# YoungSeng/QPGesture

Hardware: AMD Instinct MI355X
Metric: matched gesture frames/sec (GestureKNN) (higher is better)
Workload: dtype split-f16 products / f64 block sums + f64 re-evaluation; 1 GPU; 1 x 24 s clip (M=6 windows, Q=48 steps, 1440 frames each) per job vs speaker-10-class DB N_db=2048 windows (53248 candidates), shipped mode wavlm_feat(f32-bounded/f64-exact)+text(f32)+phase; n_db=2048, windows_per_clip=6, clips=1, clips_per_gpu=1, feature_dtype=f32, audio_precision=mixed, encode_batch=0, clips_in_flight=1, parallelism=single GPU, unsharded DB

## Files before the change

include/qpg.h:

```cpp
#ifndef QPG_H
#define QPG_H

#include <stddef.h>
#include <stdint.h>

#ifdef __cplusplus
extern "C" {
#endif

#define QPG_OK 0
#define QPG_EINVAL (-1)
#define QPG_EHIP (-2)
#define QPG_EUNSUP (-3)

typedef struct qpg_ctx qpg_ctx;

int qpg_version(void);
const char* qpg_build_id(void);
int qpg_ctx_create(int device, qpg_ctx** out);
int qpg_dev_kernarg(void);
int qpg_ctx_destroy(qpg_ctx* ctx);
#define QPG_OPT_GATE_DEDUP_FROM_CHAINS 0
#define QPG_OPT_TAKES_STAGES 1
#define QPG_OPT_NOPHASE_STAGES 2
// ... 113 lines not shown
                           int16_t* out_rank, int q_block, int64_t block_stride);
int qpg_percode_select_f32(qpg_ctx*, void* stream, const float* D, int64_t ldD, int Q, const int16_t* cand_code,
                           int64_t C, int K, float absent, int32_t idx_base, float* out_dist, int32_t* out_idx,
                           int16_t* out_rank, int q_block, int64_t block_stride);

int qpg_percode_select_guarded_f64(qpg_ctx*, void* stream, const double* D, int64_t ldD, int Q, const int16_t* cand_code,
                                   int64_t C, int K, double absent, int32_t idx_base, double* out_dist, int32_t* out_idx,
                                   int16_t* out_rank, int q_block, int64_t block_stride, const float* base, int T, int F,
                                   const int32_t* cand_t, int G, int n_taps, int tap_stride, const float* q32, double eps,
                                   int32_t* stats, int base_is_f16);

int64_t qpg_percode_select_exact_ws_bytes(int Q, int64_t C, int K);
int qpg_percode_select_exact_f64(qpg_ctx*, void* stream, const double* D, int64_t ldD, int Q, const int16_t* cand_code,
                                 int64_t C, int K, double absent, int32_t idx_base, double* out_dist, int32_t* out_idx,
                                 int16_t* out_rank, int q_block, int64_t block_stride, const float* base, int T, int F,
                                 const int32_t* cand_t, int G, int n_taps, int tap_stride, const float* q32, double eps,
                                 int32_t* stats, int base_is_f16, void* ws, int64_t ws_bytes);

int qpg_percode_select_mixed_f64(qpg_ctx*, void* stream, const void* D, int d_is_f32, int64_t ldD, int Q, const int16_t* cand_code,
                                 int64_t C, int K, double absent, int32_t idx_base, double* out_dist, int32_t* out_idx,
                                 int16_t* out_rank, int q_block, int64_t block_stride, const float* base, int T, int F,
                                 const int32_t* cand_t, int G, int n_taps, int tap_stride, const float* q32,
                                 const double* qn2, const double* cn2, double eps1, double eps2, int32_t* stats,
                                 void* ws, int64_t ws_bytes, int base_is_f16);
int64_t qpg_percode_select_mixed_ws_bytes(int Q, int K);
int64_t qpg_percode_select_mixed_ws_stride(int K);
int qpg_percode_select_mixed_f64_cut(qpg_ctx*, void* stream, const void* D, int d_is_f32, int64_t ldD, int Q,
                                     const int16_t* cand_code, int64_t C, int K, double absent, int32_t idx_base,
                                     double* out_dist, int32_t* out_idx, int16_t* out_rank, int q_block, int64_t block_stride,
                                     const float* base, int T, int F, const int32_t* cand_t, int G, int n_taps,
                                     int tap_stride, const float* q32, const double* qn2, const double* cn2, double eps1,
                                     double eps2, int32_t* stats, void* ws, int64_t ws_bytes, int base_is_f16,
                                     const int16_t* pos_rank_t, const int16_t* freq_rank, int top_n, int probe);

int64_t qpg_merge_mixed_ws_bytes(int Q, int K, int fl_cap);
int qpg_merge_mixed_phase1_f64(qpg_ctx*, void* stream, const void* recv, int W, int64_t src_stride, int64_t dist_off,
                               int64_t idx_off, int Q, int K, double absent, double eps1, int R, void* req,
                               int64_t req_stride, void* ws, int64_t ws_bytes, int32_t* stats, int fl_cap,
                               int64_t flag_off);
int qpg_shard_refine_f64(qpg_ctx*, void* stream, const void* req_recv, int W, int64_t req_stride, int R, int q_stride,
                         int64_t cand_base, const float* base, int base_is_f16, int T, int F, const int32_t* cand_t, int G,
                         int n_taps, int tap_stride, const float* q32, const double* qn2, const double* cn2, void* resp,
                         int64_t resp_stride, int reference_arithmetic, int32_t* stats, int Rq);
int qpg_flags_stamp(qpg_ctx*, void* stream, void* buf, int nblk, int64_t stride, int64_t off, const int32_t* stats);
int qpg_flags_gather(qpg_ctx*, void* stream, const void* buf, int nblk, int64_t stride, int64_t off, int32_t* stats);
int qpg_merge_mixed_phase2_f64(qpg_ctx*, void* stream, const void* recv, int W, int64_t src_stride, int64_t idx_off, int Q,
                               int K, double absent, const void* ws, int64_t ws_bytes, const void* resp_recv,
                               int64_t resp_stride, double* out_dist, int32_t* out_idx, int16_t* out_rank, int32_t* stats,
                               int fl_cap, double eps2);

int qpg_merge_select_f64(qpg_ctx*, void* stream, const void* recv, int W, int64_t src_stride, int64_t dist_off,
                         int64_t idx_off, int Q, int K, double absent, double* out_dist, int32_t* out_idx,
                         int16_t* out_rank, double eps2, int32_t* stats);
int qpg_merge_select_f32(qpg_ctx*, void* stream, const void* recv, int W, int64_t src_stride, int64_t dist_off,
                         int64_t idx_off, int Q, int K, float absent, float* out_dist, int32_t* out_idx,
                         int16_t* out_rank);

int qpg_rank_rows_f64(qpg_ctx*, void* stream, const double* d, int Q, int K, int16_t* out);
int qpg_rank_rows_f32(qpg_ctx*, void* stream, const float* d, int Q, int K, int16_t* out);


int qpg_l2_table_f32(qpg_ctx*, void* stream, const float* sig, int K, int Dm, float* out);

#define QPG_MODE_AUD_TXT 0
#define QPG_MODE_AUD 1
#define QPG_MODE_TXT 2
// ... 338 lines not shown
```

qpgesture_amd/code_knn.py:

```python
import ctypes
from collections import namedtuple
from typing import NamedTuple, Optional

import numpy as np
import torch

from . import _lib
from .parallel import allreduce_max_, allreduce_min_index, exchange_bytes, shard_rows
from .sorted_rows import SortedRows

from .constant import (ABSENT_DIST, NUM_AUDIO_FEAT_FRAMES, STEP_SZ, WAVVQ_GROUP_SIZE, codebook_size, num_frames,
                       num_frames_code)

MODE_AUD_TXT, MODE_AUD, MODE_TXT = _lib.QPG_MODE_AUD_TXT, _lib.QPG_MODE_AUD, _lib.QPG_MODE_TXT
AUDIO_MX_ERR = _lib.QPG_AUDIO_MX_ERR
AUDIO_MX_BAND = 2.1 * AUDIO_MX_ERR
AUDIO_HL_ERR = _lib.QPG_AUDIO_HL_ERR
AUDIO_HL_BAND = 2.1 * AUDIO_HL_ERR

FLAG_LIST_OVERFLOW, FLAG_SMALL_NORMS, FLAG_REQUEST_OVERFLOW, FLAG_CROSS_SHARD_TIE = 1, 2, 4, 8
FLAG_TEXT_OVERFLOW = 16


_PIN_SENTINEL = -1234567
# ... 227 lines not shown
        from . import db_cache
        return db_cache.save(self, path, key, sources=sources)

    @classmethod
    def load(cls, path, device="cuda:0", key=None):
        from . import db_cache
        dev = torch.device(device)
        if dev.type != "cuda":
            raise RuntimeError("GestureDB needs a HIP device (got %s); there is no CPU path" % dev)
        _lib.load()
        db = db_cache.load(path, dev, key)
        if db is None:
            return None
        if db.hl_image is not None or db.txt_sorted is not None:
            from .selfcheck import mfma_bound_ok
            db.hl_bound_ok, db.hl_bound_report = mfma_bound_ok(dev)
            if not db.hl_bound_ok:
                db.hl_image = db.txt_sorted = None
        return db

    @staticmethod
    def _cand_code(code_local, cidx, dev):
        cc = np.ascontiguousarray(code_local[:, np.asarray(cidx, np.int64)].reshape(-1))
        cc = np.where((cc >= 0) & (cc < 32767), cc, -1).astype(np.int16)
        return torch.from_numpy(cc if cc.size else np.zeros((1,), np.int16)).to(dev)

    @property
    def idx_base(self):
        return self.lo


Knobs = namedtuple("Knobs", "audio_precision audio_kernel text_kernel tie_eps mixed_single_launch sharded_mixed "
                   "sharded_mixed_min_gflop force_sharded overlap_sweeps text_after_sweep audio_first fused_pack rank_cut "
                   "split_fuse split_fuse_max_steps host_ranks use_wavvq",
                   defaults=("mixed", "hl", "mfma", 1e-12, False, True, 20.0, False, True, True, None, True, True, True,
                             256, False, False))
DBFacts = namedtuple("DBFacts", "n_local N world K Ga F Dt feature_dtype hl_bound_ok has_hl_image has_txt_sorted hl_planes",
                     defaults=("f32", True, True, True, 2))


class AudioPlan(NamedTuple):
    path: str
    kernel: str
    band: float
    cut_top_n: int
    fused_rank: bool


class StepPlan(NamedTuple):
    audio: Optional[AudioPlan]
    text: Optional[str]
    sharded: bool
    exchange: Optional[str]
    clip_pack: bool
    split_fuse: bool
    overlap: bool
    order: Optional[str]


def plan_audio(kn, db, Q, want_rank=False, reduce=True, out_given=False, cut_top_n=0):
    C = db.n_local * db.Ga
    fused_rank = want_rank and db.world == 1
    local_final = fused_rank and reduce and not out_given
    shard_part = (db.world > 1 or kn.force_sharded) and not reduce and out_given
    gflop = 2e-9 * Q * (-(-db.N // db.world) * db.Ga) * NUM_AUDIO_FEAT_FRAMES * db.F
    guard = kn.tie_eps > 0 and C > 0
    half = db.feature_dtype == "f16"
    if (kn.audio_precision == "mixed" and guard and db.K <= 512 and db.hl_bound_ok and
            (local_final or (shard_part and kn.sharded_mixed and gflop >= kn.sharded_mixed_min_gflop))):
        hl = kn.audio_kernel == "hl" and db.has_hl_image
        kernel = ("hl" if db.hl_planes == 2 else "hl1") if hl else ("mx_h" if half else "mx")
        cut = cut_top_n if (cut_top_n in (1, 2) and local_final and not kn.mixed_single_launch) else 0
        return AudioPlan("mixed", kernel, AUDIO_HL_BAND if hl else AUDIO_MX_BAND, cut, fused_rank)
    path = "exact" if (kn.audio_precision == "exact" and guard) else ("guarded" if guard else "plain")
    return AudioPlan(path, "f64_h" if half else "f64", 0.0, 0, fused_rank)


def plan_text(kn, db, Q, reduce=True, out_given=False):
    mfma = (kn.text_kernel == "mfma" and db.has_txt_sorted and Q > 0 and kn.audio_precision != "exact" and
            ((not out_given and reduce and db.world == 1) or (out_given and not reduce)))
    return "mfma" if mfma else "valu"


def plan_step(kn, db, M, steps, mode=MODE_AUD_TXT, for_walk=False, owner_blocks=False):
    Q = M * steps
    sharded = db.world > 1 or kn.force_sharded
    audio = text = None
    if mode != MODE_TXT and not kn.use_wavvq:
        cut = 0
        if for_walk and kn.rank_cut and not sharded and not kn.host_ranks:
            cut = 1 if mode == MODE_AUD_TXT else 2
        audio = plan_audio(kn, db, Q, want_rank=not sharded, reduce=not sharded, out_given=sharded, cut_top_n=cut)
    if mode != MODE_AUD:
        text = plan_text(kn, db, Q, reduce=not sharded, out_given=sharded)
    split = (for_walk and mode == MODE_AUD_TXT and not sharded and not kn.host_ranks and kn.split_fuse and
             db.K % 16 == 0 and db.K <= 4096 and Q <= kn.split_fuse_max_steps)
    overlap = mode == MODE_AUD_TXT and kn.overlap_sweeps
    mfma_text = kn.text_kernel == "mfma" and db.has_txt_sorted and kn.audio_precision != "exact"
    clip_pack = (overlap and not kn.use_wavvq and mfma_text and audio.kernel in ("hl", "hl1") and db.Dt % 128 == 0 and
                 kn.fused_pack)
    audio_first = mfma_text if kn.audio_first is None else bool(kn.audio_first)
    after = overlap and kn.text_after_sweep and not audio_first and not kn.use_wavvq
    order = None
    if overlap:
        order = "audio_first" if audio_first else ("text_after_sweep" if after else "text_first")
    exchange = ("all_to_all" if owner_blocks else "all_gather") if sharded else None
    return StepPlan(audio, text, sharded, exchange, clip_pack, split, overlap, order)

# ... 62 lines not shown
        if use_wavvq and not db.has_wavvq:
            raise ValueError("GestureDB was built without a wavvq track")
        self.db = db
        self.use_wavvq = use_wavvq
        if use_wavvq:
            self.step_sz, self.n_db_frm = db.vq_step, db.Tv
        else:
            self.step_sz, self.n_db_frm = db.step_sz, db.T
        self.n_db_seq = db.N
        self.use_phase, self.use_txt = use_phase, use_txt
        if not use_phase and not 0 <= int(desired_k) < _lib.QPG_NOPHASE_KMAX:
            raise ValueError("desired_k must be in [0, %d) (got %r)" % (_lib.QPG_NOPHASE_KMAX, desired_k))
        self.desired_k = int(desired_k)
        self.last_picks = None
        self.rng = rng if rng is not None else np.random
        self.overlap_sweeps = True
        self.text_after_sweep = True
        self.audio_first = None
        self.serial_walk = False
        self.tie_eps = 1e-12
        self._guard_stats = torch.zeros((4,), dtype=torch.int32, device=db.device)
        self.audio_precision = "mixed"
        self.audio_kernel = "hl"
        self.text_kernel = "mfma"
        self._txt_scratch = {}
        self.fallbacks = 0
        import os as _os
        self.fused_pack = _os.environ.get("QPG_FUSED_PACK", "1") != "0"
        self.rank_cut = _os.environ.get("QPG_RANK_CUT", "1") != "0"
        self.rank_cut_probe = 64
        self.mixed_single_launch = False
        self.split_fuse = True
        self.split_fuse_max_steps = 256
        self.sharded_mixed = True
        self.force_sharded = False
        self.sharded_mixed_min_gflop = 20.0
        self.mixed_requests = None
        self.host_ranks = False

        self._qpos, self._qcache, self._layouts, self._mm_cache, self._pinned_ints, self._plans = None, {}, {}, {}, {}, {}
        self._side_stream = self._side_gate = self._side_done = self._sweep_event = None
        self._mix_ws = self._exact_ws = self._hl_qimage = self._takes_ws = self._nophase_ws = None
        self._pinned_nophase = None
        self.kernel_events, self.kernel_events_every, self.kernel_event_pool, self._ev_calls = None, 1, None, 0
        self.text_fallbacks, self.tables, self._last_mix_Q = 0, None, 0
        self._last_audio_mixed = self._last_audio_exact = self._last_audio_hl = False
        self._last_text_mfma = self._last_rank_cut = False
        self._last_D_aud = self._last_q32 = self._last_qn2 = self._last_ints = self._last_gate_tables = None

    def _knobs(self):
        return Knobs(self.audio_precision, self.audio_kernel, self.text_kernel, self.tie_eps, self.mixed_single_launch,
                     self.sharded_mixed, self.sharded_mixed_min_gflop, self.force_sharded, self.overlap_sweeps,
                     self.text_after_sweep, self.audio_first, self.fused_pack, self.rank_cut, self.split_fuse,
                     self.split_fuse_max_steps, self.host_ranks, self.use_wavvq)

    def _facts(self):
        db = self.db
        return DBFacts(db.n_local, db.N, db.world, db.K, db.Ga, db.F, db.Dt, db.feature_dtype, db.hl_bound_ok,
                       db.hl_image is not None, db.txt_sorted is not None, db.hl_planes)

    def _audio_grid(self):
        db = self.db
        if self.use_wavvq:
            return db.vq_cidx, db.vq_pslot, db.Gv
        return db.aud_cidx, db.aud_pslot, db.Ga

    def query_positions(self):
        key = (self.n_db_frm, self.step_sz)
        if self._qpos is not None and self._qpos[0] == key:
            return self._qpos[1]
        pos, i = [], 0
        while i < self.n_db_frm:
            pos.append(i)
            i += STEP_SZ * self.step_sz
        self._qpos = (key, pos)
        return pos

    def init_code_phase(self):
        db = self.db
        i = self.rng.randint(0, self.n_db_seq)
        j = self.rng.randint(0, self.n_db_frm - int(num_frames / num_frames_code))
        code = int(db.code_host[i, j // num_frames_code])
        if not self.use_phase:
            return code
        P = db.phase_host[i, j:j + 8]
        if P.shape[0] != 8:
            raise ValueError("init_code_phase drew frame %d: phase slice has %d rows, not 8 "
# ... 65 lines not shown
        else:
            assert prepacked is None, "the one-launch clip pack feeds the split-f16 sweep only"
            _lib.call("qpg_audio_pack_queries", dev, qbase, M, T, F, _i32(q_win, dev), _i32(q_t, dev), Q,
                      NUM_AUDIO_FEAT_FRAMES, ts, q32, qn2)
        if timer is not None:
            timer[0].record(torch.cuda.current_stream(dev))
        if use_hl:
            sweep_launch()
        else:
            strides = (1, D.stride(0), self._guard_stats) if mixed else (D.stride(0),)
            _lib.call(sweep_fn, dev, db.base, db.n_local, db.T, db.F, db.aud_t, db.Ga, NUM_AUDIO_FEAT_FRAMES,
                      db.tap_stride, db.cn2, q32, qn2, Q, D, *strides)
        if timer is not None:
            timer[1].record(torch.cuda.current_stream(dev))
            self.kernel_events.append(timer)
        if after_sweep is not None:
            after_sweep()
        if sweep_event is not None:
            sweep_event.record(torch.cuda.current_stream(dev))
        if plan.path == "plain":
            dist, idx, rank = self._select_plain(D, db.aud_cand_code, C, db.Ga, out, plan.fused_rank)
        else:
            dist, idx, rank, qb, bs = self._tables_out(Q, torch.float64, out, plan.fused_rank)
            tables = (Q, db.aud_cand_code, C, db.K, float(ABSENT_DIST), db.idx_base * db.Ga, dist, idx, rank, qb, bs)
            track = (db.base, db.T, db.F, db.aud_t, db.Ga, NUM_AUDIO_FEAT_FRAMES, db.tap_stride, q32)
        if mixed:
            ws = self._mix_ws = _grown(self._mix_ws, int(_lib.load().qpg_percode_select_mixed_ws_bytes(Q, db.K)), dev,
                                       zero=True)
            single = self.mixed_single_launch
            sel_args = (D, 1, D.stride(0), *tables, *track, qn2, db.cn2, plan.band, float(self.tie_eps),
                        self._guard_stats, None if single else ws, 0 if single else ws.numel(), int(half))
            try:
                if plan.cut_top_n:
                    _lib.call("qpg_percode_select_mixed_f64_cut", dev, *sel_args, db.pos_rank_t, db.freq_rank,
                              int(plan.cut_top_n), int(self.rank_cut_probe))
                else:
                    _lib.call("qpg_percode_select_mixed_f64", dev, *sel_args)
            except Exception:
                self._mix_ws = None
                raise
        elif plan.path == "exact":
            ws = self._exact_ws = _grown(self._exact_ws, int(_lib.load().qpg_percode_select_exact_ws_bytes(Q, C, db.K)),
                                         dev)
            _lib.call("qpg_percode_select_exact_f64", dev, D, D.stride(0), *tables, *track, float(self.tie_eps),
                      self._guard_stats, int(half), ws, ws.numel())
        elif plan.path == "guarded":
            _lib.call("qpg_percode_select_guarded_f64", dev, D, D.stride(0), *tables, *track, float(self.tie_eps),
                      self._guard_stats, int(half))
        self._last_audio_mixed, self._last_audio_exact, self._last_audio_hl = mixed, plan.path == "exact", use_hl
        self._last_rank_cut, self._last_D_aud, self._last_q32, self._last_qn2 = plan.cut_top_n > 0, D, q32, qn2
        if mixed:
            self._last_mix_Q = Q
        return AudioResult(dist, idx, rank, D, q32, qn2, plan)

    def sweep_text(self, queries, want_rank=False, reduce=True, normalised=False, out=None, cols_packed=False, kind=None):
        db, dev = self.db, self.db.device
        Q = queries.shape[0]
        if normalised:
            qn = queries
        else:
            qn = torch.empty_like(queries)
            _lib.call("qpg_l2_normalize_rows_f32", dev, queries, Q, db.Dt, qn)
        if kind is None:
            kind = plan_text(self._knobs(), self._facts(), Q, reduce, out is not None)
        self._last_text_mfma = kind == "mfma"
        if kind == "mfma":
            dist, idx, rank, qb, bs = self._tables_out(Q, torch.float32, out, want_rank and out is None)
            db.txt_sorted.select(qn, float(ABSENT_DIST), self._guard_stats, dist=dist, idx=idx, rank=rank,
# ... 579 lines not shown
```

qpgesture_amd/csrc/qpg_select.hip:

```cpp
#include "qpg_common.h"

__device__ __forceinline__ unsigned long long order_key(double d) {
  unsigned long long b = (unsigned long long)__double_as_longlong(d);
  return (b >> 63) ? ~b : (b | 0x8000000000000000ull);
}
__device__ __forceinline__ double key_value(unsigned long long k, double) {
  unsigned long long b = (k >> 63) ? (k & 0x7fffffffffffffffull) : ~k;
  return __longlong_as_double((long long)b);
}
__device__ __forceinline__ unsigned int order_key(float d) {
  unsigned int b = __float_as_uint(d);
  return (b >> 31) ? ~b : (b | 0x80000000u);
}
__device__ __forceinline__ float key_value(unsigned int k, float) {
  unsigned int b = (k >> 31) ? (k & 0x7fffffffu) : ~k;
  return __uint_as_float(b);
}

template <typename T, typename KeyT, bool PACKED>
__global__ __launch_bounds__(1024) void percode_select_kernel(const T* __restrict__ D, int64_t ldD,
                                                              const int16_t* __restrict__ cand_code, int64_t C, int K,
                                                              T absent, int32_t idx_base, T* __restrict__ out_dist,
                                                              int32_t* __restrict__ out_idx,
                                                              int16_t* __restrict__ out_rank, int q_block,
// ... 392 lines not shown
      [&]() {
        if (tid == 0) A.stats[1] = 1;
      },
      rank_pass);
}

extern "C" int qpg_percode_select_guarded_f64(qpg_ctx* ctx, void* stream, const double* D, int64_t ldD, int Q,
                                              const int16_t* cand_code, int64_t C, int K, double absent,
                                              int32_t idx_base, double* out_dist, int32_t* out_idx, int16_t* out_rank,
                                              int q_block, int64_t block_stride, const float* base, int T, int F,
                                              const int32_t* cand_t, int G, int n_taps, int tap_stride,
                                              const float* q32, double eps, int32_t* stats, int base_is_f16) {
  const char* name = "qpg_percode_select_guarded_f64";
  QPG_REQUIRE(ctx && D && (cand_code || C == 0) && out_dist && out_idx && base && cand_t && q32 && stats,
              "%s: null pointer", name);
  QPG_REQUIRE(Q >= 0 && C >= 0 && K > 0 && K <= 2048 && ldD >= C && C + (int64_t)idx_base < 0x7fffffffll && eps >= 0.0,
              "%s: bad size (K <= 2048)", name);
  QPG_REQUIRE(select_block_layout_ok(q_block, block_stride, Q, out_rank), QPG_BLOCK_LAYOUT_MSG, name);
  GuardArgs A;
  if (int rc = guard_args(name, &A, base, base_is_f16, q32, cand_t, T, F, G, n_taps, tap_stride, C, eps, stats)) return rc;
  if (Q == 0) return QPG_OK;
  size_t sh = 24 * (size_t)K + GUARD_LIST * 16 + 16;
  const int sort_ranks = sh + 12 * (size_t)rank_sort_pow2(K) <= 64 * 1024;
  if (sort_ranks) sh += 12 * (size_t)rank_sort_pow2(K);
  hipLaunchKernelGGL(percode_select_guarded_f64_kernel, dim3(Q), dim3(1024), sh, qpg_stream(stream), D, ldD, cand_code,
                     C, K, absent, idx_base, out_dist, out_idx, out_rank, q_block, block_stride, A, sort_ranks);
  QPG_LAUNCH_CHECK("percode_select_guarded_f64_kernel");
  return QPG_OK;
}

#define MIX_LIST 2048
#define MIX_LIST2 256
#define MIX_POT 6144

template <int NPER>
__device__ __forceinline__ double pair_dot_fast_f64(const GuardArgs& A, const float* qlds, int64_t c_local, int lane) {
  const int j = (int)(c_local / A.G), g = (int)(c_local - (int64_t)j * A.G);
  const int t0 = A.cand_t[g];
  const int64_t crow = (int64_t)j * A.T * A.F + lane * 4;
  f32x4 cv[6][NPER];
#pragma unroll
  for (int tap = 0; tap < 6; ++tap) {
    const int t = t0 + tap * A.tap_stride;
    const bool ok = t < A.T;
    const int64_t cp = crow + (int64_t)(ok ? t : t0) * A.F;
#pragma unroll
    for (int u = 0; u < NPER; ++u) {
      cv[tap][u] = guard_val4(A, cp + 256 * u);
      if (!ok) cv[tap][u] = (f32x4){0.f, 0.f, 0.f, 0.f};
    }
  }
  double s0 = 0.0, s1 = 0.0;
#pragma unroll
  for (int tap = 0; tap < 6; ++tap)
#pragma unroll
    for (int u = 0; u < NPER; ++u) {
      const f32x4 qv = *reinterpret_cast<const f32x4*>(qlds + tap * A.F + 256 * u + lane * 4);
      s0 += (double)qv.x * (double)cv[tap][u].x;
      s1 += (double)qv.y * (double)cv[tap][u].y;
      s0 += (double)qv.z * (double)cv[tap][u].z;
      s1 += (double)qv.w * (double)cv[tap][u].w;
    }
  double s = s0 + s1;
  for (int o = 32; o > 0; o >>= 1) s += __shfl_xor(s, o, 64);
  return s;
}
// ... 157 lines not shown
        if (key[u][e] < o) o = atomicMin(&best32[code], key[u][e]);
        const unsigned int lo = o < key[u][e] ? o : key[u][e];
        if ((double)d[u][e] <= (double)key_value(lo, 0.f) + eps1) {
          const int pp = atomicAdd(&n_pot, 1);
          if (pp < MIX_SPOT) {
            pc[pp] = (int)(b + (int64_t)u * blockDim.x * 4 + e);
            pd[pp] = d[u][e];
            pk[pp] = (int16_t)code;
          }
        }
      }
  }
  for (int64_t c = cv + tid; c < c1; c += blockDim.x) visit(c, row[c], cand_code[c]);
  __syncthreads();
  MixStream m = mix_stream_of(ws, q, K);
  for (int k = tid; k < K; k += blockDim.x) m.inv[(size_t)sl * K + k] = ~best32[k];
  const int np = n_pot;
  if (np > MIX_SPOT) {
    if (tid == 0) m.cnt[sl] = -1;
    return;
  }
  const int seg = sl * MIX_SPOT;
  for (int e = tid; e < np; e += blockDim.x) {
    if (!((double)pd[e] <= (double)key_value(best32[pk[e]], 0.f) + eps1)) continue;
    const int pos = seg + atomicAdd(&n_keep, 1);
    m.pot_c[pos] = pc[e];
    m.pot_d[pos] = pd[e];
    m.pot_k[pos] = pk[e];
  }
  __syncthreads();
  if (tid == 0) m.cnt[sl] = n_keep;
}

template <typename DT>
__global__ __launch_bounds__(1024) void percode_select_mixed_f64_kernel(
    const DT* __restrict__ D, int64_t ldD, const int16_t* __restrict__ cand_code, int64_t C, int K, double absent,
    int32_t idx_base, double* __restrict__ out_dist, int32_t* __restrict__ out_idx, int16_t* __restrict__ out_rank,
    int q_block, int64_t block_stride, GuardArgs A, double eps1, const double* __restrict__ cn2,
    const double* __restrict__ qn2, int use_qlds, int phase, unsigned char* __restrict__ ws, int pre, RankCut RC) {
  extern __shared__ __attribute__((aligned(16))) unsigned char smem[];
  unsigned long long* best = reinterpret_cast<unsigned long long*>(smem);
  double* v = reinterpret_cast<double*>(smem + 8 * (size_t)K);
  unsigned int* besti = reinterpret_cast<unsigned int*>(smem + 16 * (size_t)K);
  unsigned int* near_ = besti + K;
  int* s_code = reinterpret_cast<int*>(near_ + K);
  unsigned char* refd = reinterpret_cast<unsigned char*>(s_code + K);
  unsigned char* tail = smem + 32 * (size_t)K;
  double* l_d = reinterpret_cast<double*>(tail);
  int* l_c = reinterpret_cast<int*>(tail + 8 * MIX_LIST);
  int* l_k = l_c + MIX_LIST;
  int* l2 = l_k + MIX_LIST;
  int* ctl = l2 + MIX_LIST2;
  int* p_c = ctl + 8;
  int16_t* p_k = reinterpret_cast<int16_t*>(p_c + MIX_LIST);
  int* rk = reinterpret_cast<int*>(p_k + MIX_LIST);
  int* pot_c = rk + K;
  int16_t* pot_k = reinterpret_cast<int16_t*>(pot_c + MIX_POT);
  float* qlds = reinterpret_cast<float*>(pot_k + MIX_POT);
  const int q = blockIdx.x, tid = threadIdx.x, lane = tid & 63, wv = tid >> 6, nwv = blockDim.x >> 6;
  const DT* row = D + (int64_t)q * ldD;
  select_out_rows(q, K, q_block, block_stride, out_dist, out_idx);
  unsigned char* wq = ws ? mix_query_base(ws, q, K) : nullptr;
  for (int k = tid; k < K; k += blockDim.x) {
    best[k] = ~0ull;
    besti[k] = 0xffffffffu;
    near_[k] = 0;
    refd[k] = 0;
// ... 138 lines not shown
    for (int e = tid; e < npot; e += blockDim.x) pass2(pot_c[e], (double)row[pot_c[e]], pot_k[e]);
  } else {
#pragma unroll 4
    for (int64_t c = (int64_t)tid * VE; c < Cv; c += (int64_t)blockDim.x * VE) {
      const vecD d = *reinterpret_cast<const vecD*>(row + c);
      const vecC cd = *reinterpret_cast<const vecC*>(cand_code + c);
#pragma unroll
      for (int e = 0; e < VE; ++e) pass2(c + e, (double)d[e], cd[e]);
    }
    for (int64_t c = Cv + tid; c < C; c += blockDim.x) pass2(c, (double)row[c], cand_code[c]);
  }
  __syncthreads();
  if (streamed && tid < MIX_SPLIT) ms.cnt[tid] = 0;
  for (int k = tid; k < K; k += blockDim.x) v[k] = besti[k] != 0xffffffffu ? key_value(best[k], 0.0) : absent;
  __syncthreads();
  const bool cut = RC.pos_t != nullptr && streamed && out_rank != nullptr && phase == 1;
  unsigned char* need2 = nullptr;
  if (cut) {
    unsigned char* cs = reinterpret_cast<unsigned char*>(pot_c);
    const int Kp = rank_sort_pow2(K);
    unsigned long long* skey2 = reinterpret_cast<unsigned long long*>(cs);
    int* scode2 = reinterpret_cast<int*>(skey2 + Kp);
    int16_t* lo_ = reinterpret_cast<int16_t*>(scode2 + Kp);
    int16_t* hi_ = lo_ + K;
    unsigned char* need = reinterpret_cast<unsigned char*>(hi_ + K);
    need2 = need + K;
    double* red = reinterpret_cast<double*>(cs + 12 * (size_t)Kp + 8 * (size_t)((K + 7) / 8 * 8));
    const double f05 = tid < K ? (double)RC.freq[tid] * 0.05 : 0.0;
    block_sorted_ranks(v, K, skey2, scode2, [&](int k, int r) {
      s_code[r] = k;
      rk[k] = r;
    });
    __syncthreads();
    for (int r = tid; r < K; r += blockDim.x) reinterpret_cast<int16_t*>(wq + mix_park_order_off(K))[r] = (int16_t)s_code[r];
    order_parked = true;
    for (int r = tid; r < K; r += blockDim.x) {
      const int k = s_code[r];
      int b = 0, a = 0;
      if (besti[k] != 0xffffffffu) {
        while (r - 1 - b >= 0 && v[k] - v[s_code[r - 1 - b]] <= eps1) ++b;
        while (r + 1 + a < K && besti[s_code[r + 1 + a]] != 0xffffffffu && v[s_code[r + 1 + a]] - v[k] <= eps1) ++a;
      }
      lo_[k] = (int16_t)(r - b);
      hi_[k] = (int16_t)(r + a);
    }
    __syncthreads();
    int np = RC.probe < K ? RC.probe : K;
    np = np < 64 ? np : 64;
    double* pf_ = red + 17;
    double* ph_ = pf_ + 64;
    int* pk_ = reinterpret_cast<int*>(ph_ + 64);
    double* pm_ = reinterpret_cast<double*>(pk_ + 64);
    if (tid < K) pm_[tid] = f05;
    __syncthreads();
    for (int r = tid; r < 64; r += blockDim.x) {
      const int k = r < np ? s_code[r] : -1;
      const bool ok = k >= 0 && besti[k] != 0xffffffffu;
      pk_[r] = ok ? k : -1;
      pf_[r] = ok ? pm_[k] : 0.0;
      ph_[r] = ok ? (double)hi_[k] : 0.0;
    }
    __syncthreads();
    double u = -1.0, m1 = __builtin_inf(), m2 = __builtin_inf();
    const int pp = tid < K ? tid : tid - K, half = tid < K ? 0 : 1;
    if (tid < 2 * K) {
      const int r0 = 32 * half;
      int kk[32];
// ... 108 lines not shown
      const long long b = (long long)floor(v[k] * inv_w);
      const unsigned int s0 = slot(b);
      bool company = false;
#pragma unroll
      for (int o = -1; o <= 1; ++o) {
        const unsigned int si = slot(b + o);
        if (o != 0 && si == s0) continue;
        unsigned int c = cell[si];
        if (si == s0) c -= 0x10000u + (unsigned int)k;
        const unsigned int pop = c >> 16;
        if (pop == 1) {
          const int other = (int)(c & 0xffffu);
          company |= fabs(v[other] - v[k]) < eps1;
        } else if (pop > 1) {
          company = true;
        }
      }
      if (!company || (need2 && !need2[k])) continue;
      if (atomicMax(&near_[k], 2u) >= 2u) continue;
      const int pos = atomicAdd(&ctl[0], 1);
      if (pos < MIX_LIST) {
        l_c[pos] = (int)(besti[k] - (unsigned int)idx_base);
        l_k[pos] = k;
      }
    }
    __syncthreads();
  }
  n = ctl[0];
  if (n > MIX_LIST) {
    n = MIX_LIST;
    if (tid == 0) atomicOr(&A.stats[1], 1);
  }
  }
  if (phase == 1) {
    unsigned long long* w_best = reinterpret_cast<unsigned long long*>(wq);
    double* w_v = reinterpret_cast<double*>(wq + 8 * (size_t)K);
    unsigned int* w_bi = reinterpret_cast<unsigned int*>(wq + 16 * (size_t)K);
    unsigned int* w_nr = w_bi + K;
    int* w_n = reinterpret_cast<int*>(wq + 24 * (size_t)K);
    int* w_lc = w_n + 4;
    int* w_lk = w_lc + MIX_LIST;
    for (int k = tid; k < K; k += blockDim.x) {
      w_best[k] = best[k];
      w_v[k] = v[k];
      w_bi[k] = besti[k];
      w_nr[k] = near_[k];
    }
    for (int e = tid; e < n; e += blockDim.x) {
      w_lc[e] = l_c[e];
      w_lk[e] = l_k[e];
    }
    if (tid == 0) {
      w_n[0] = n;
      w_n[1] = order_parked ? 1 : 0;
    }
    return;
  }
  if (phase == 2) {
    const unsigned long long* w_best = reinterpret_cast<const unsigned long long*>(wq);
    const double* w_v = reinterpret_cast<const double*>(wq + 8 * (size_t)K);
    const unsigned int* w_bi = reinterpret_cast<const unsigned int*>(wq + 16 * (size_t)K);
    const unsigned int* w_nr = w_bi + K;
    const int* w_n = reinterpret_cast<const int*>(wq + 24 * (size_t)K);
    const int* w_lc = w_n + 4;
    const int* w_lk = w_lc + MIX_LIST;
    const double* w_ld = reinterpret_cast<const double*>(w_lk + MIX_LIST);
    n = w_n[0];
    for (int k = tid; k < K; k += blockDim.x) {
      best[k] = w_best[k];
      v[k] = w_v[k];
      besti[k] = w_bi[k];
      near_[k] = w_nr[k];
    }
    for (int e = tid; e < n; e += blockDim.x) {
      l_c[e] = w_lc[e];
      l_k[e] = w_lk[e];
      l_d[e] = w_ld[e];
    }
    if (RC.pos_t) {
      unsigned char* isref = reinterpret_cast<unsigned char*>(pot_c);
      for (int k = tid; k < K; k += blockDim.x) isref[k] = 0;
      __syncthreads();
      for (int e = tid; e < n; e += blockDim.x) isref[w_lk[e]] = 1;
    }
    __syncthreads();
  }
  if (n > 0) {
    const double qq = qn2[q];
    const bool fast = use_qlds != 0;
    if (phase == 0 && fast) {
      const int D4 = (A.n_taps * A.F) >> 2;
      const f32x4* src = reinterpret_cast<const f32x4*>(A.q32 + (int64_t)q * A.n_taps * A.F);
      for (int i = tid; i < D4; i += blockDim.x) reinterpret_cast<f32x4*>(qlds)[i] = src[i];
      __syncthreads();
    }
    for (int e = wv; e < n && phase == 0; e += nwv) {
      const double d = pair_distance_wave(A, q, qlds, l_c[e], lane, fast, qq, cn2);
      if (lane == 0) l_d[e] = d;
    }
    for (int k = tid; k < K; k += blockDim.x)
      if (near_[k] >= 2) {
        rk[k] = (int)besti[k];
        best[k] = ~0ull;
        besti[k] = 0xffffffffu;
        s_code[k] = 0;
      }
    __syncthreads();
    for (int e = tid; e < n; e += blockDim.x) atomicMin(&best[l_k[e]], (unsigned long long)order_key(l_d[e]));
    __syncthreads();
    if (A.eps > 0.0) {
      for (int e = tid; e < n; e += blockDim.x)
        if (l_d[e] <= key_value(best[l_k[e]], 0.0) + A.eps) atomicAdd(&s_code[l_k[e]], 1);
      __syncthreads();
      for (int e = tid; e < n; e += blockDim.x)
        if (s_code[l_k[e]] >= 2 && l_d[e] <= key_value(best[l_k[e]], 0.0) + A.eps) {
          const int pos = atomicAdd(&ctl[2], 1);
          if (pos < MIX_LIST2) l2[pos] = e;
        }
      __syncthreads();
      int n2 = ctl[2];
      if (n2 > MIX_LIST2) {
        n2 = MIX_LIST2;
        if (tid == 0) atomicOr(&A.stats[1], 1);
      }
      if (n2 > 0) {
        for (int i0 = 0; i0 < n2; i0 += blockDim.x / 4) {
          const int i = i0 + (tid >> 2);
          const int e = l2[i < n2 ? i : 0];
          const double dr = refine_pair_f64(A, q, l_c[e], tid & 3);
// ... 3 lines not shown
          }
        }
        __syncthreads();
        for (int k = tid; k < K; k += blockDim.x)
          if (refd[k]) best[k] = ~0ull;
        __syncthreads();
        for (int i = tid; i < n2; i += blockDim.x)
          atomicMin(&best[l_k[l2[i]]], (unsigned long long)order_key(l_d[l2[i]]));
        __syncthreads();
        if (tid == 0) atomicAdd(&A.stats[0], n2);
      }
    }
    for (int e = tid; e < n; e += blockDim.x)
      if ((unsigned long long)order_key(l_d[e]) == best[l_k[e]])
        atomicMin(&besti[l_k[e]], (unsigned int)(l_c[e] + idx_base));
    __syncthreads();
    for (int k = tid; k < K; k += blockDim.x)
      if (near_[k] >= 2) {
        if (best[k] != ~0ull) v[k] = key_value(best[k], 0.0);
        else besti[k] = (unsigned int)rk[k];
      }
    if (tid == 0) atomicAdd(&A.stats[2], n);
    __syncthreads();
  }
  for (int k = tid; k < K; k += blockDim.x) {
    const bool have = besti[k] != 0xffffffffu;
    out_dist[(int64_t)q * K + k] = v[k];
    out_idx[(int64_t)q * K + k] = have ? (int32_t)besti[k] : -1;
  }
  if (!out_rank) return;
  if (tid == 0) ctl[2] = 0;
  __syncthreads();
  bool repaired = false;
  if (phase == 2 && RC.pos_t && reinterpret_cast<const int*>(wq + 24 * (size_t)K)[1] == 1) {
    const int16_t* w_order = reinterpret_cast<const int16_t*>(wq + mix_park_order_off(K));
    for (int r = tid; r < K; r += blockDim.x) s_code[r] = w_order[r];
    __syncthreads();
    for (int round = 0; round < 24 && !repaired; ++round) {
      if (tid == 0) ctl[5] = 0;
      __syncthreads();
#pragma unroll
      for (int parity = 0; parity < 2; ++parity) {
        for (int r = 2 * tid + parity; r + 1 < K; r += 2 * blockDim.x) {
          const int ka = s_code[r], kb = s_code[r + 1];
          if (rank_gt(rank_sort_key(v[ka]), ka, rank_sort_key(v[kb]), kb)) {
            s_code[r] = kb;
            s_code[r + 1] = ka;
            ctl[5] = 1;
          }
        }
        __syncthreads();
      }
      repaired = ctl[5] == 0;
      __syncthreads();
    }
    if (repaired)
      for (int r = tid; r < K; r += blockDim.x) out_rank[(int64_t)q * K + s_code[r]] = (int16_t)r;
  }
  if (!repaired) rank_pass(true);
  if (A.eps <= 0.0) return;
  __syncthreads();
  for (int r = tid; r + 1 < K; r += blockDim.x) {
    const int ka = s_code[r], kb = s_code[r + 1];
    if (besti[ka] == 0xffffffffu || besti[kb] == 0xffffffffu) continue;
    if (phase == 2 && RC.pos_t &&
        !(reinterpret_cast<const unsigned char*>(pot_c)[ka] && reinterpret_cast<const unsigned char*>(pot_c)[kb]))
      continue;
    if (v[kb] - v[ka] < A.eps) {
#pragma unroll
      for (int h = 0; h < 2; ++h) {
        const int k = h ? kb : ka;
        if (atomicExch(&near_[k], 0xffffffffu) == 0xffffffffu || refd[k]) continue;
        const int pos = atomicAdd(&ctl[2], 1);
        if (pos < MIX_LIST2) {
          l2[pos] = k;
        }
      }
    }
  }
  __syncthreads();
  int n3 = ctl[2];
  if (n3 == 0) return;
  if (n3 > MIX_LIST2) {
    n3 = MIX_LIST2;
    if (tid == 0) atomicOr(&A.stats[1], 1);
  }
  for (int i0 = 0; i0 < n3; i0 += blockDim.x / 4) {
    const int i = i0 + (tid >> 2);
    const int k = l2[i < n3 ? i : 0];
    const double dr = refine_pair_f64(A, q, (int64_t)(besti[k] - (unsigned int)idx_base), tid & 3);
    if (i < n3 && (tid & 3) == 0) {
      v[k] = dr;
      out_dist[(int64_t)q * K + k] = dr;
    }
  }
  if (tid == 0) atomicAdd(&A.stats[0], n3);
  __syncthreads();
  rank_pass(true);
}

extern "C" int64_t qpg_percode_select_mixed_ws_bytes(int Q, int K) {
  return (Q <= 0 || K <= 0) ? 0 : (int64_t)((size_t)Q * mix_ws_stride(K));
}
extern "C" int64_t qpg_percode_select_mixed_ws_stride(int K) {
  return K <= 0 ? 0 : (int64_t)mix_ws_stride(K);
}

static int select_mixed_impl(const char* name, qpg_ctx* ctx, void* stream, const void* D, int d_is_f32, int64_t ldD, int Q,
                             const int16_t* cand_code, int64_t C, int K, double absent,
                             int32_t idx_base, double* out_dist, int32_t* out_idx, int16_t* out_rank,
                             int q_block, int64_t block_stride, const float* base, int T, int F,
                             const int32_t* cand_t, int G, int n_taps, int tap_stride,
                             const float* q32, const double* qn2, const double* cn2, double eps1,
                             double eps2, int32_t* stats, void* ws, int64_t ws_bytes, int base_is_f16,
                             const RankCut* cut = nullptr) {
  QPG_REQUIRE(ctx && D && (cand_code || C == 0) && out_dist && out_idx && base && cand_t && q32 && qn2 && cn2 && stats,
              "%s: null pointer", name);
  QPG_REQUIRE(Q >= 0 && C >= 0 && K > 0 && K <= 512 && ldD >= C && C + (int64_t)idx_base < 0x7fffffffll,
              "%s: bad size (K <= 512)", name);
  QPG_REQUIRE((F % 4) == 0 && eps1 >= 2.0 * QPG_AUDIO_HL_ERR && eps2 >= 0.0 && eps2 < eps1,
              "%s: bad geometry (F %% 4 == 0) or eps (eps1 >= 2 x the sweep's error bound - at least %g -, 0 <= eps2 < eps1)",
              name, 2.0 * (double)QPG_AUDIO_HL_ERR);
  QPG_REQUIRE(select_block_layout_ok(q_block, block_stride, Q, out_rank), QPG_BLOCK_LAYOUT_MSG, name);
  GuardArgs A;
  if (int rc = guard_args(name, &A, base, base_is_f16, q32, cand_t, T, F, G, n_taps, tap_stride, C, eps2, stats)) return rc;
  if (Q == 0) return QPG_OK;
  const int use_qlds = (n_taps == 6 && F == 1024) ? 1 : 0;
  const size_t sh2 = 32 * (size_t)K + 16 * MIX_LIST + 4 * MIX_LIST2 + 32 + 6 * MIX_LIST + 4 * (size_t)K;
  size_t sh2c = sh2;
  const RankCut RCnone = {nullptr, nullptr, 1, 0};
  const size_t sh1 = sh2 + 6 * MIX_POT;
  const size_t sh = sh1 + (use_qlds ? (size_t)n_taps * F * 4 : 0);
  if (!ctx->select_lds_raised) {
    if (hipFuncSetAttribute(reinterpret_cast<const void*>(percode_select_mixed_f64_kernel<double>),
                            hipFuncAttributeMaxDynamicSharedMemorySize, 128 * 1024) != hipSuccess ||
        hipFuncSetAttribute(reinterpret_cast<const void*>(percode_select_mixed_f64_kernel<float>),
                            hipFuncAttributeMaxDynamicSharedMemorySize, 128 * 1024) != hipSuccess) {
      qpg_set_error("%s: cannot raise the dynamic LDS limit", name);
      return QPG_EHIP;
    }
    ctx->select_lds_raised = true;
  }
  unsigned char* w = static_cast<unsigned char*>(ws);
  if (ws)
    QPG_REQUIRE(ws_bytes >= qpg_percode_select_mixed_ws_bytes(Q, K) && (reinterpret_cast<uintptr_t>(ws) % 16) == 0,
                "%s: workspace too small or misaligned (qpg_percode_select_mixed_ws_bytes)", name);
#define SEL_MIX_LAUNCH(DT, SH, PHASE, PRE)                                                                                  \
  hipLaunchKernelGGL((percode_select_mixed_f64_kernel<DT>), dim3(Q), dim3(1024), SH, qpg_stream(stream),               \
                     static_cast<const DT*>(D), ldD, cand_code, C, K, absent, idx_base, out_dist, out_idx, out_rank,   \
                     q_block, block_stride, A, eps1, cn2, qn2, use_qlds, PHASE, w, PRE, RCv)
  RankCut RCv = RCnone;
  if (!ws) {
    if (d_is_f32) SEL_MIX_LAUNCH(float, sh, 0, 0); else SEL_MIX_LAUNCH(double, sh, 0, 0);
    QPG_LAUNCH_CHECK("percode_select_mixed_f64_kernel");
    return QPG_OK;
  }
  if (d_is_f32) {
    const size_t shs = 4 * (size_t)K + 10 * (size_t)MIX_SPOT;
    hipLaunchKernelGGL(mixed_stream_kernel, dim3(Q, MIX_SPLIT), dim3(1024), shs, qpg_stream(stream),
                       static_cast<const float*>(D), ldD, cand_code, C, K, eps1, w);
    QPG_LAUNCH_CHECK("mixed_stream_kernel");
    if (cut && cut->pos_t && out_rank) {
      RCv = *cut;
      sh2c = sh2 + 12 * (size_t)rank_sort_pow2(K) + 8 * (size_t)((K + 7) / 8 * 8) + 17 * 8 + 64 * (8 + 8 + 4) +
             16 * (size_t)K;
    }
    SEL_MIX_LAUNCH(float, sh2c, 1, 1);
  } else {
    SEL_MIX_LAUNCH(double, sh1, 1, 0);
  }
  QPG_LAUNCH_CHECK("percode_select_mixed_f64_kernel (lists)");
  const int rb = Q >= 512 ? 8 : (Q >= 128 ? 16 : 64);
  hipLaunchKernelGGL((select_refine_kernel<4>), dim3(Q, rb), dim3(256), 0, qpg_stream(stream), A, K, cn2, qn2, w, use_qlds);
  QPG_LAUNCH_CHECK("select_refine_kernel");
  if (d_is_f32) SEL_MIX_LAUNCH(float, sh2c, 2, 0); else SEL_MIX_LAUNCH(double, sh2, 2, 0);
  QPG_LAUNCH_CHECK("percode_select_mixed_f64_kernel (merge)");
#undef SEL_MIX_LAUNCH
  return QPG_OK;
}

extern "C" int qpg_percode_select_mixed_f64(qpg_ctx* ctx, void* stream, const void* D, int d_is_f32, int64_t ldD, int Q,
                                            const int16_t* cand_code, int64_t C, int K, double absent,
                                            int32_t idx_base, double* out_dist, int32_t* out_idx, int16_t* out_rank,
                                            int q_block, int64_t block_stride, const float* base, int T, int F,
                                            const int32_t* cand_t, int G, int n_taps, int tap_stride,
                                            const float* q32, const double* qn2, const double* cn2, double eps1,
                                            double eps2, int32_t* stats, void* ws, int64_t ws_bytes, int base_is_f16) {
  return select_mixed_impl("qpg_percode_select_mixed_f64", ctx, stream, D, d_is_f32, ldD, Q, cand_code, C, K, absent, idx_base,
                           out_dist, out_idx, out_rank, q_block, block_stride, base, T, F, cand_t, G, n_taps, tap_stride, q32,
                           qn2, cn2, eps1, eps2, stats, ws, ws_bytes, base_is_f16);
}

extern "C" int qpg_percode_select_mixed_f64_cut(qpg_ctx* ctx, void* stream, const void* D, int d_is_f32, int64_t ldD, int Q,
                                                const int16_t* cand_code, int64_t C, int K, double absent,
                                                int32_t idx_base, double* out_dist, int32_t* out_idx, int16_t* out_rank,
                                                int q_block, int64_t block_stride, const float* base, int T, int F,
                                                const int32_t* cand_t, int G, int n_taps, int tap_stride,
                                                const float* q32, const double* qn2, const double* cn2, double eps1,
                                                double eps2, int32_t* stats, void* ws, int64_t ws_bytes, int base_is_f16,
                                                const int16_t* pos_rank_t, const int16_t* freq_rank, int top_n, int probe) {
  const char* name = "qpg_percode_select_mixed_f64_cut";
  QPG_REQUIRE(pos_rank_t && freq_rank && out_rank && ws && d_is_f32 && q_block == 0 && (top_n == 1 || top_n == 2) &&
                  probe >= 0,
              "%s: needs the rank tables, out_rank, an f32 matrix, a workspace, no block layout, top_n 1 or 2", name);
  RankCut rc = {pos_rank_t, freq_rank, top_n, probe > 0 ? probe : 64};
  return select_mixed_impl(name, ctx, stream, D, d_is_f32, ldD, Q, cand_code, C, K, absent, idx_base, out_dist, out_idx,
                           out_rank, q_block, block_stride, base, T, F, cand_t, G, n_taps, tap_stride, q32, qn2, cn2, eps1, eps2,
                           stats, ws, ws_bytes, base_is_f16, &rc);
}

template <typename T, typename KeyT, bool PACKED>
static int percode_select(const char* name, qpg_ctx* ctx, void* stream, const T* D, int64_t ldD, int Q,
                          const int16_t* cand_code, int64_t C, int K, T absent, int32_t idx_base, T* out_dist,
                          int32_t* out_idx, int16_t* out_rank, int q_block, int64_t block_stride) {
  QPG_REQUIRE(ctx && D && (cand_code || C == 0) && out_dist && out_idx, "%s: null pointer", name);
  QPG_REQUIRE(Q >= 0 && C >= 0 && K > 0 && K <= 2048 && ldD >= C && C + (int64_t)idx_base < 0x7fffffffll,
              "%s: bad size (K <= 2048, candidate indices must stay below 2^31)", name);
  QPG_REQUIRE(select_block_layout_ok(q_block, block_stride, Q, out_rank), QPG_BLOCK_LAYOUT_MSG, name);
  if (Q == 0) return QPG_OK;
  const size_t sh = 12 * (size_t)rank_sort_pow2(K) + (size_t)K * sizeof(T);
  hipLaunchKernelGGL((percode_select_kernel<T, KeyT, PACKED>), dim3(Q), dim3(1024), sh, qpg_stream(stream), D, ldD,
                     cand_code, C, K, absent, idx_base, out_dist, out_idx, out_rank, q_block, block_stride);
  QPG_LAUNCH_CHECK(name);
  return QPG_OK;
}

extern "C" int qpg_percode_select_f64(qpg_ctx* ctx, void* stream, const double* D, int64_t ldD, int Q,
                                      const int16_t* cand_code, int64_t C, int K, double absent, int32_t idx_base,
                                      double* out_dist, int32_t* out_idx, int16_t* out_rank, int q_block,
                                      int64_t block_stride) {
  return percode_select<double, unsigned long long, false>("qpg_percode_select_f64", ctx, stream, D, ldD, Q, cand_code,
                                                           C, K, absent, idx_base, out_dist, out_idx, out_rank, q_block,
                                                           block_stride);
}
extern "C" int qpg_percode_select_f32(qpg_ctx* ctx, void* stream, const float* D, int64_t ldD, int Q,
                                      const int16_t* cand_code, int64_t C, int K, float absent, int32_t idx_base,
                                      float* out_dist, int32_t* out_idx, int16_t* out_rank, int q_block,
                                      int64_t block_stride) {
  return percode_select<float, unsigned int, true>("qpg_percode_select_f32", ctx, stream, D, ldD, Q, cand_code, C, K,
                                                   absent, idx_base, out_dist, out_idx, out_rank, q_block, block_stride);
}
// ... 691 lines not shown
```

Baseline: 5.179 million frames/s.

## Fuse rank-cut mixed select into a two-launch finish kernel for short queries

Adds a FINISH template variant of the mixed-precision per-code select kernel. When the step count is at most a new knob (default 48), this variant parks the rank order in LDS, computes pair distances itself and performs the rank-cut repair inside a single block per query. The three later launches (list, refine, merge) are skipped. This is meant to cut launch and global-workspace round-trip overhead for small Q. In exchange, each block does all refinement serially, which can be slower when there are many candidates per query.

```diff
diff --git a/include/qpg.h b/include/qpg.h
--- a/include/qpg.h
+++ b/include/qpg.h
@@ -169,6 +169,14 @@
                                      int tap_stride, const float* q32, const double* qn2, const double* cn2, double eps1,
                                      double eps2, int32_t* stats, void* ws, int64_t ws_bytes, int base_is_f16,
                                      const int16_t* pos_rank_t, const int16_t* freq_rank, int top_n, int probe);
+int qpg_percode_select_mixed_f64_cut_finish(qpg_ctx*, void* stream, const void* D, int d_is_f32, int64_t ldD, int Q,
+                                            const int16_t* cand_code, int64_t C, int K, double absent, int32_t idx_base,
+                                            double* out_dist, int32_t* out_idx, int16_t* out_rank, int q_block,
+                                            int64_t block_stride, const float* base, int T, int F, const int32_t* cand_t,
+                                            int G, int n_taps, int tap_stride, const float* q32, const double* qn2,
+                                            const double* cn2, double eps1, double eps2, int32_t* stats, void* ws,
+                                            int64_t ws_bytes, int base_is_f16, const int16_t* pos_rank_t,
+                                            const int16_t* freq_rank, int top_n, int probe);
 
 int64_t qpg_merge_mixed_ws_bytes(int Q, int K, int fl_cap);
 int qpg_merge_mixed_phase1_f64(qpg_ctx*, void* stream, const void* recv, int W, int64_t src_stride, int64_t dist_off,
diff --git a/qpgesture_amd/code_knn.py b/qpgesture_amd/code_knn.py
--- a/qpgesture_amd/code_knn.py
+++ b/qpgesture_amd/code_knn.py
@@ -283,9 +283,9 @@
 
 Knobs = namedtuple("Knobs", "audio_precision audio_kernel text_kernel tie_eps mixed_single_launch sharded_mixed "
                    "sharded_mixed_min_gflop force_sharded overlap_sweeps text_after_sweep audio_first fused_pack rank_cut "
-                   "split_fuse split_fuse_max_steps host_ranks use_wavvq",
+                   "split_fuse split_fuse_max_steps host_ranks use_wavvq finish_select_max_steps",
                    defaults=("mixed", "hl", "mfma", 1e-12, False, True, 20.0, False, True, True, None, True, True, True,
-                             256, False, False))
+                             256, False, False, 48))
 DBFacts = namedtuple("DBFacts", "n_local N world K Ga F Dt feature_dtype hl_bound_ok has_hl_image has_txt_sorted hl_planes",
                      defaults=("f32", True, True, True, 2))
 
@@ -325,6 +325,16 @@
         return AudioPlan("mixed", kernel, AUDIO_HL_BAND if hl else AUDIO_MX_BAND, cut, fused_rank)
     path = "exact" if (kn.audio_precision == "exact" and guard) else ("guarded" if guard else "plain")
     return AudioPlan(path, "f64_h" if half else "f64", 0.0, 0, fused_rank)
+
+
+def plan_select_launches(kn, plan, Q):
+    if plan.path != "mixed":
+        return 1 if plan.path in ("guarded", "plain") else 5
+    if kn.mixed_single_launch:
+        return 1
+    if plan.cut_top_n and 0 < Q <= kn.finish_select_max_steps:
+        return 2
+    return 4
 
 
 def plan_text(kn, db, Q, reduce=True, out_given=False):
@@ -453,6 +463,7 @@
         self.mixed_single_launch = False
         self.split_fuse = True
         self.split_fuse_max_steps = 256
+        self.finish_select_max_steps = 48
         self.sharded_mixed = True
         self.force_sharded = False
         self.sharded_mixed_min_gflop = 20.0
@@ -473,7 +484,7 @@
         return Knobs(self.audio_precision, self.audio_kernel, self.text_kernel, self.tie_eps, self.mixed_single_launch,
                      self.sharded_mixed, self.sharded_mixed_min_gflop, self.force_sharded, self.overlap_sweeps,
                      self.text_after_sweep, self.audio_first, self.fused_pack, self.rank_cut, self.split_fuse,
-                     self.split_fuse_max_steps, self.host_ranks, self.use_wavvq)
+                     self.split_fuse_max_steps, self.host_ranks, self.use_wavvq, self.finish_select_max_steps)
 
     def _facts(self):
         db = self.db
@@ -605,8 +616,9 @@
                         self._guard_stats, None if single else ws, 0 if single else ws.numel(), int(half))
             try:
                 if plan.cut_top_n:
-                    _lib.call("qpg_percode_select_mixed_f64_cut", dev, *sel_args, db.pos_rank_t, db.freq_rank,
-                              int(plan.cut_top_n), int(self.rank_cut_probe))
+                    two = plan_select_launches(self._knobs(), plan, Q) == 2
+                    _lib.call("qpg_percode_select_mixed_f64_cut" + ("_finish" if two else ""), dev, *sel_args,
+                              db.pos_rank_t, db.freq_rank, int(plan.cut_top_n), int(self.rank_cut_probe))
                 else:
                     _lib.call("qpg_percode_select_mixed_f64", dev, *sel_args)
             except Exception:
diff --git a/qpgesture_amd/csrc/qpg_select.hip b/qpgesture_amd/csrc/qpg_select.hip
--- a/qpgesture_amd/csrc/qpg_select.hip
+++ b/qpgesture_amd/csrc/qpg_select.hip
@@ -448,6 +448,8 @@
 #define MIX_LIST 2048
 #define MIX_LIST2 256
 #define MIX_POT 6144
+#define MIX_FINISH_ORDER_OFF (6 * MIX_POT - 1024)
+static_assert(12 * 512 + 8 * 512 + 17 * 8 + 64 * (8 + 8 + 4) + 16 * 512 <= MIX_FINISH_ORDER_OFF, "the cut's scratch reaches the order");
 
 template <int NPER>
 __device__ __forceinline__ double pair_dot_fast_f64(const GuardArgs& A, const float* qlds, int64_t c_local, int lane) {
@@ -671,7 +673,7 @@
   if (tid == 0) m.cnt[sl] = n_keep;
 }
 
-template <typename DT>
+template <typename DT, bool FINISH = false>
 __global__ __launch_bounds__(1024) void percode_select_mixed_f64_kernel(
     const DT* __restrict__ D, int64_t ldD, const int16_t* __restrict__ cand_code, int64_t C, int K, double absent,
     int32_t idx_base, double* __restrict__ out_dist, int32_t* __restrict__ out_idx, int16_t* __restrict__ out_rank,
@@ -876,7 +878,11 @@
       rk[k] = r;
     });
     __syncthreads();
-    for (int r = tid; r < K; r += blockDim.x) reinterpret_cast<int16_t*>(wq + mix_park_order_off(K))[r] = (int16_t)s_code[r];
+    if constexpr (FINISH) {
+      for (int r = tid; r < K; r += blockDim.x) reinterpret_cast<int16_t*>(cs + MIX_FINISH_ORDER_OFF)[r] = (int16_t)s_code[r];
+    } else {
+      for (int r = tid; r < K; r += blockDim.x) reinterpret_cast<int16_t*>(wq + mix_park_order_off(K))[r] = (int16_t)s_code[r];
+    }
     order_parked = true;
     for (int r = tid; r < K; r += blockDim.x) {
       const int k = s_code[r];
@@ -1051,7 +1057,15 @@
     if (tid == 0) atomicOr(&A.stats[1], 1);
   }
   }
-  if (phase == 1) {
+  if constexpr (FINISH) {
+    if (tid == 0) reinterpret_cast<int*>(wq + 24 * (size_t)K)[0] = n;
+    unsigned char* isref = reinterpret_cast<unsigned char*>(pot_c);
+    for (int k = tid; k < K; k += blockDim.x) isref[k] = 0;
+    __syncthreads();
+    for (int e = tid; e < n; e += blockDim.x) isref[l_k[e]] = 1;
+    __syncthreads();
+  }
+  if (!FINISH && phase == 1) {
     unsigned long long* w_best = reinterpret_cast<unsigned long long*>(wq);
     double* w_v = reinterpret_cast<double*>(wq + 8 * (size_t)K);
     unsigned int* w_bi = reinterpret_cast<unsigned int*>(wq + 16 * (size_t)K);
@@ -1107,13 +1121,14 @@
   if (n > 0) {
     const double qq = qn2[q];
     const bool fast = use_qlds != 0;
-    if (phase == 0 && fast) {
+    const bool own_pairs = FINISH || phase == 0;
+    if (own_pairs && fast) {
       const int D4 = (A.n_taps * A.F) >> 2;
       const f32x4* src = reinterpret_cast<const f32x4*>(A.q32 + (int64_t)q * A.n_taps * A.F);
       for (int i = tid; i < D4; i += blockDim.x) reinterpret_cast<f32x4*>(qlds)[i] = src[i];
       __syncthreads();
     }
-    for (int e = wv; e < n && phase == 0; e += nwv) {
+    for (int e = wv; e < n && own_pairs; e += nwv) {
       const double d = pair_distance_wave(A, q, qlds, l_c[e], lane, fast, qq, cn2);
       if (lane == 0) l_d[e] = d;
     }
@@ -1183,8 +1198,10 @@
   if (tid == 0) ctl[2] = 0;
   __syncthreads();
   bool repaired = false;
-  if (phase == 2 && RC.pos_t && reinterpret_cast<const int*>(wq + 24 * (size_t)K)[1] == 1) {
-    const int16_t* w_order = reinterpret_cast<const int16_t*>(wq + mix_park_order_off(K));
+  if (FINISH ? order_parked
+             : (phase == 2 && RC.pos_t && reinterpret_cast<const int*>(wq + 24 * (size_t)K)[1] == 1)) {
+    const int16_t* w_order = FINISH ? reinterpret_cast<const int16_t*>(reinterpret_cast<unsigned char*>(pot_c) + MIX_FINISH_ORDER_OFF)
+                                    : reinterpret_cast<const int16_t*>(wq + mix_park_order_off(K));
     for (int r = tid; r < K; r += blockDim.x) s_code[r] = w_order[r];
     __syncthreads();
     for (int round = 0; round < 24 && !repaired; ++round) {
@@ -1214,7 +1231,7 @@
   for (int r = tid; r + 1 < K; r += blockDim.x) {
     const int ka = s_code[r], kb = s_code[r + 1];
     if (besti[ka] == 0xffffffffu || besti[kb] == 0xffffffffu) continue;
-    if (phase == 2 && RC.pos_t &&
+    if ((FINISH || phase == 2) && RC.pos_t &&
         !(reinterpret_cast<const unsigned char*>(pot_c)[ka] && reinterpret_cast<const unsigned char*>(pot_c)[kb]))
       continue;
     if (v[kb] - v[ka] < A.eps) {
@@ -1264,7 +1281,7 @@
                              const int32_t* cand_t, int G, int n_taps, int tap_stride,
                              const float* q32, const double* qn2, const double* cn2, double eps1,
                              double eps2, int32_t* stats, void* ws, int64_t ws_bytes, int base_is_f16,
-                             const RankCut* cut = nullptr) {
+                             const RankCut* cut = nullptr, bool finish = false) {
   QPG_REQUIRE(ctx && D && (cand_code || C == 0) && out_dist && out_idx && base && cand_t && q32 && qn2 && cn2 && stats,
               "%s: null pointer", name);
   QPG_REQUIRE(Q >= 0 && C >= 0 && K > 0 && K <= 512 && ldD >= C && C + (int64_t)idx_base < 0x7fffffffll,
@@ -1286,6 +1303,8 @@
     if (hipFuncSetAttribute(reinterpret_cast<const void*>(percode_select_mixed_f64_kernel<double>),
                             hipFuncAttributeMaxDynamicSharedMemorySize, 128 * 1024) != hipSuccess ||
         hipFuncSetAttribute(reinterpret_cast<const void*>(percode_select_mixed_f64_kernel<float>),
+                            hipFuncAttributeMaxDynamicSharedMemorySize, 128 * 1024) != hipSuccess ||
+        hipFuncSetAttribute(reinterpret_cast<const void*>(percode_select_mixed_f64_kernel<float, true>),
                             hipFuncAttributeMaxDynamicSharedMemorySize, 128 * 1024) != hipSuccess) {
       qpg_set_error("%s: cannot raise the dynamic LDS limit", name);
       return QPG_EHIP;
@@ -1315,6 +1334,13 @@
       RCv = *cut;
       sh2c = sh2 + 12 * (size_t)rank_sort_pow2(K) + 8 * (size_t)((K + 7) / 8 * 8) + 17 * 8 + 64 * (8 + 8 + 4) +
              16 * (size_t)K;
+    }
+    if (finish) {
+      hipLaunchKernelGGL((percode_select_mixed_f64_kernel<float, true>), dim3(Q), dim3(1024), sh, qpg_stream(stream),
+                         static_cast<const float*>(D), ldD, cand_code, C, K, absent, idx_base, out_dist, out_idx, out_rank,
+                         q_block, block_stride, A, eps1, cn2, qn2, use_qlds, 1, w, 1, RCv);
+      QPG_LAUNCH_CHECK("percode_select_mixed_f64_kernel (finish)");
+      return QPG_OK;
     }
     SEL_MIX_LAUNCH(float, sh2c, 1, 1);
   } else {
@@ -1358,6 +1384,25 @@
   return select_mixed_impl(name, ctx, stream, D, d_is_f32, ldD, Q, cand_code, C, K, absent, idx_base, out_dist, out_idx,
                            out_rank, q_block, block_stride, base, T, F, cand_t, G, n_taps, tap_stride, q32, qn2, cn2, eps1, eps2,
                            stats, ws, ws_bytes, base_is_f16, &rc);
+}
+
+extern "C" int qpg_percode_select_mixed_f64_cut_finish(qpg_ctx* ctx, void* stream, const void* D, int d_is_f32, int64_t ldD,
+                                                       int Q, const int16_t* cand_code, int64_t C, int K, double absent,
+                                                       int32_t idx_base, double* out_dist, int32_t* out_idx, int16_t* out_rank,
+                                                       int q_block, int64_t block_stride, const float* base, int T, int F,
+                                                       const int32_t* cand_t, int G, int n_taps, int tap_stride,
+                                                       const float* q32, const double* qn2, const double* cn2, double eps1,
+                                                       double eps2, int32_t* stats, void* ws, int64_t ws_bytes, int base_is_f16,
+                                                       const int16_t* pos_rank_t, const int16_t* freq_rank, int top_n,
+                                                       int probe) {
+  const char* name = "qpg_percode_select_mixed_f64_cut_finish";
+  QPG_REQUIRE(pos_rank_t && freq_rank && out_rank && ws && d_is_f32 && q_block == 0 && (top_n == 1 || top_n == 2) &&
+                  probe >= 0,
+              "%s: needs the rank tables, out_rank, an f32 matrix, a workspace, no block layout, top_n 1 or 2", name);
+  RankCut rc = {pos_rank_t, freq_rank, top_n, probe > 0 ? probe : 64};
+  return select_mixed_impl(name, ctx, stream, D, d_is_f32, ldD, Q, cand_code, C, K, absent, idx_base, out_dist, out_idx,
+                           out_rank, q_block, block_stride, base, T, F, cand_t, G, n_taps, tap_stride, q32, qn2, cn2, eps1, eps2,
+                           stats, ws, ws_bytes, base_is_f16, &rc, true);
 }
 
 template <typename T, typename KeyT, bool PACKED>
```

Result: no change. 5.223 million frames/s (median of 2 runs) (+0.9%).
